# PhilippBongartz/RepeatResolver

Measured on AMD Instinct MI355X. Metric: sum-of-pairs DP cells/sec, higher is better.
Workload: dtype u32

## Files before the change

repeatresolver_amd/csrc/pwr_device.hip:

```cpp
#include <hip/hip_runtime.h>

#include <algorithm>
#include <chrono>
#include <cstdint>
#include <cstdio>
#include <cstdlib>
#include <cstring>
#include <new>
#include <thread>
#include <type_traits>
#include <vector>

#include "pwr.h"

#define PWR_INF 0x40000000u
#define PWR_BIG 0x7fffffff

struct Hdr {
    int W;
    int nslots;
    int nfree;
    int cur;
    int status;
    int stop;
// ... 990 lines not shown
                }
            } else {
                unsigned Mn[C];
                unsigned fa = 0;
#pragma unroll
                for (int i = 0; i < C; ++i) {
                    fa |= (tg[i] >= p) ? (1u << i) : 0u;
                    p = min(p, tg[i]);
                    Mn[i] = (rel0 + i < 0) ? PWR_INF : (unsigned)(gg[i] + p);
                }
                const unsigned mrow = needP ? ePy : PWR_INF;
                const unsigned left0 = (unsigned)__builtin_amdgcn_update_dpp((int)mrow, (int)Mn[C - 1], DPP_WAVE_SHR1, 0xF, 0xF, false);
#pragma unroll
                for (int i = 0; i < C; ++i) {
                    const unsigned lf = i ? Mn[i > 0 ? i - 1 : 0] : left0;
                    const bool inb = (unsigned)(rel0 + i) < (unsigned)Bx;
                    accA[i] = (accA[i] << 1) | ((((fa >> i) & 1u) || (inb && Mn[i] == lf)) ? 1u : 0u);
                    lastM[wave * MS + lc + i] = inb ? Mn[i] : 0xffffffffu;
                    Mprev[i] = Mn[i];
                }
            }
            nacc = (x & 15) + 1;
            if (lane == 63) {
                ST64(MBP(wave, x), P_end, x + 1);
                ST64(MBM(wave, x), Mprev[C - 1], x + 1);
                if (ms == ms_hi) ST64(PTB(x), P_end, x + 1);
            }
            ran_prev = 1;
            V2_NEXT_ROW()
        }
        if (lane == 0) __hip_atomic_store(&rdone[wave], round + 1, __ATOMIC_RELAXED, __HIP_MEMORY_SCOPE_WORKGROUP);
        __syncthreads();
        if (UNI(__hip_atomic_load(&s_done, __ATOMIC_RELAXED, __HIP_MEMORY_SCOPE_WORKGROUP)) >= NW) break;
    }
    if (round >= max_rounds) {
        if (tid == 0) { m->ok = 0; atomicCAS(&st.hdr->status, 0, PWR_ERR_INTERNAL); }
        return;
    }
    if (tid == 0) {
        m->clk = (unsigned)(__builtin_amdgcn_s_memtime() - t_clk0);
        m->rclk = (unsigned)(__builtin_amdgcn_s_memrealtime() - t_real0);
        m->rounds = round;
        atomicAdd(&st.hdr->cells_computed, m->cells);
    }
#undef MBP
#undef MBM
#undef PTB
#undef LD64
#undef LD32LO
#undef ST64
}

#ifndef PWR_INTERIOR_CLS
#define PWR_INTERIOR_CLS 0
#endif
#define V3_TICKS() ((unsigned)(__builtin_amdgcn_s_memtime() >> 10))
#define V3_TIMEOUT_TICKS (1u << 19)
#define V4_RB 128

#ifdef PWR_DIAG
#define DG_DECL unsigned long long dg_wait_fast = 0, dg_wait_gen = 0, dg_wait_setup = 0, dg_t = 0, dg_t2 = 0, dg_cyc_int = 0, dg_cyc_gen16 = 0, dg_ts1 = 0, dg_ts2 = 0, dg_tl2 = 0; unsigned dg_log = 0; unsigned dg_int = 0, dg_gen16 = 0, dg_general = 0, dg_nowork = 0, dg_runs = 0, dg_switch = 0;
#define DG_T0() dg_t = __builtin_amdgcn_s_memtime();
#define DG_ADD(ACC) ACC += __builtin_amdgcn_s_memtime() - dg_t;
#define DG_INC(CNT, N) CNT += (N);
#define DG_T2() dg_t2 = __builtin_amdgcn_s_memtime();
#define DG_ADD2(ACC) ACC += __builtin_amdgcn_s_memtime() - dg_t2;
#else
#define DG_T2()
#define DG_ADD2(ACC)
#define DG_DECL
#define DG_T0()
#define DG_ADD(ACC)
#define DG_INC(CNT, N)
#endif
template <int NW, int C, bool WG1>
__global__ __launch_bounds__(WG1 ? NW * 64 : 128) void k_fill_v3(DState st, JobBufs jb)
{
    constexpr int MS = 64 * C, RS = NW * MS;
    constexpr int NL = WG1 ? NW : 1;
    constexpr int RB = WG1 ? 64 : V4_RB;
    __shared__ __attribute__((aligned(16))) int ldsS1[NL][2][4][MS];
    __shared__ unsigned long long rP[NL][RB], rM[NL][RB];
    __shared__ int wprog[NL], wdone;
    const int vjob = WG1 ? (int)blockIdx.x : (int)(blockIdx.x + 8 * blockIdx.z), lane = threadIdx.x & 63;
    const int role = WG1 ? 0 : UNI((int)threadIdx.x >> 6);
    const int wave = WG1 ? UNI((int)threadIdx.x >> 6) : (int)blockIdx.y;
    const int lw = WG1 ? wave : 0, wr = WG1 ? (wave + 1) % NW : 0;
    if (vjob >= jb.njobs_launched * jb.smax) return;
    const int job = vjob / jb.smax;
    const SegDesc *const sd = jb.seg + (size_t)job * SEG_MAX + (vjob % jb.smax);
    JobMeta *m = &jb.meta[job];
    if (st.hdr->fallback > 0 && jb.v2_follows) return;
    if (!m->active || m->L <= 0 || !m->ok || m->wide || !sd->active || NOT_MINE(jb, job)) return;
    const int seg_xb = UNI(sd->xb), seg_fin = UNI(sd->fin);
    const int L = UNI(sd->xe) - seg_xb;
    const int Lf = seg_fin ? L - 1 : L;
    const int x_own = UNI(sd->xown) - seg_xb;
    const int g_own = x_own >> 4;
    const int chkA = x_own > 0 ? x_own : -1, chkB = seg_fin ? -1 : L;
    unsigned *const chk_w = jb.chk + (((size_t)job * (SEG_MAX + 1) + sd->s) * 2 + 0) * (size_t)jb.NC;
    unsigned *const chk_t = jb.chk + (((size_t)job * (SEG_MAX + 1) + sd->s + 1) * 2 + 1) * (size_t)jb.NC;
    const unsigned long long t_clk0 = __builtin_amdgcn_s_memtime(), t_real0 = __builtin_amdgcn_s_memrealtime();
    for (int i = threadIdx.x; i < NL * RB; i += blockDim.x) { (&rP[0][0])[i] = 0; (&rM[0][0])[i] = 0; }
    if (threadIdx.x < NL) wprog[threadIdx.x] = 0;
    if (threadIdx.x == 0) wdone = 0;
    __syncthreads();

    const int wl = (wave + NW - 1) % NW;
    const unsigned tagbase = jb.tagbase;
    const size_t gstride = (size_t)jb.gstride;
    unsigned long long *const gmy = jb.gmb + (((size_t)job * NW + wave) * gstride + (size_t)sd->grow0) * 2;
    const unsigned long long *const gleftw = jb.gmb + (((size_t)job * NW + wl) * gstride + (size_t)sd->grow0) * 2;
    const unsigned long long *const gjob = jb.gmb + ((size_t)job * NW * gstride + (size_t)sd->grow0) * 2;
#define PTOT_PTR(AP, BP, R) (gjob + (((size_t)((((AP) + (BP) - 1 - lo) / MS) % NW)) * gstride + (size_t)(R)) * 2)
    int *const abortf = &m->abort;
#define GLD(PTR) __hip_atomic_load((PTR), __ATOMIC_RELAXED, __HIP_MEMORY_SCOPE_AGENT)
#define GST(PTR, VAL, ROW) __hip_atomic_store((PTR), ((unsigned long long)(tagbase | (unsigned)((ROW) + 1)) << 32) | (unsigned)(VAL), __ATOMIC_RELAXED, __HIP_MEMORY_SCOPE_AGENT)
#define GST2(PTR, VAL, TAG) __hip_atomic_store((PTR), ((unsigned long long)(TAG) << 32) | (unsigned)(VAL), __ATOMIC_RELAXED, __HIP_MEMORY_SCOPE_AGENT)
#define TAGOF(W64) ((unsigned)((W64) >> 32))
#define LLD(REF) __hip_atomic_load(&(REF), __ATOMIC_RELAXED, __HIP_MEMORY_SCOPE_WORKGROUP)
#define LST(REF, V) __hip_atomic_store(&(REF), (V), __ATOMIC_RELAXED, __HIP_MEMORY_SCOPE_WORKGROUP)

    if (!WG1 && role == 1) {
        for (unsigned it = 0;; ++it) {
            if (UNI(LLD(wdone))) break;
            const int wx = UNI(LLD(wprog[lw]));
            const int r = wx - 1 + lane;
            const bool inr = r >= 0 && r < L;
            unsigned long long p = 0, q = 0;
            int ab = 0;
            if (inr) { p = GLD(gleftw + 2 * (size_t)r); q = GLD(gleftw + 2 * (size_t)r + 1); }
            if ((it & 15u) == 15u) ab = GLD(abortf);
            if (inr) {
                const unsigned tagr = tagbase | (unsigned)(r + 1);
                if (TAGOF(p) == tagr && TAGOF(q) == tagr) {
                    LST(rP[lw][r & (RB - 1)], p);
                    __hip_atomic_store(&rM[lw][r & (RB - 1)], q, __ATOMIC_RELEASE, __HIP_MEMORY_SCOPE_WORKGROUP);
                }
            }
            if (UNI(ab)) break;
        }
        return;
    }

    const int lo = UNI(m->lo), hi = UNI(m->hi), W = UNI(m->W), B = st.B, H = st.H;
    const int *way = jb.way + (size_t)job * jb.Lmax + seg_xb;
    const uint8_t *seq = st.seq + st.rowoff[UNI(m->k)] + seg_xb;
    const int4 *rec2 = jb.rec2 + (size_t)job * jb.colcap * 2;
    uint32_t *dirs = jb.dirs + (size_t)job * jb.dirstride + (size_t)(seg_xb >> 4) * RS;
    unsigned *lastM = jb.lastM + (size_t)job * jb.NC;
    const int lc = lane * C;
#define V4_LOADS(MSX, SLOT, AU, AG, AI, GL)                                                      \
    {                                                                                            \
        _Pragma("unroll") for (int i = 0; i < C; ++i) {                                          \
            const int y_ = lo + (MSX) * MS + lc + i;                                             \
            int4 p_ = make_int4(PWR_BIG / 2, PWR_BIG / 2, PWR_BIG / 2, PWR_BIG / 2);             \
            int4 q_ = make_int4(PWR_BIG / 2, 0, PWR_BIG / 2, 0);                                 \
            if (y_ <= hi) { p_ = rec2[2 * (y_ - lo)]; q_ = rec2[2 * (y_ - lo) + 1]; }            \
            ldsS1[lw][SLOT][0][lc + i] = p_.x; ldsS1[lw][SLOT][1][lc + i] = p_.y;                        \
            ldsS1[lw][SLOT][2][lc + i] = p_.z; ldsS1[lw][SLOT][3][lc + i] = p_.w;                        \
            AU[i] = q_.x; AG[i] = q_.y; AI[i] = q_.z;                                            \
        }                                                                                        \
        const int yq_ = lo + (MSX) * MS - 1;                                                     \
        GL = (yq_ >= lo && yq_ <= hi) ? UNI(rec2[2 * (yq_ - lo) + 1].y) : 0;                     \
    }

    int ug[C], gg[C], ig[C];
    int nu[C], ng[C], ni[C];
    int gleft = 0, gleftn = 0;
    const int ms_first = (max(0, UNI(way[0]) - H) - lo) / MS;
    int ms = ms_first + (((wave - ms_first) % NW) + NW) % NW, msn = ms + NW;
    int cs = 0;
    V4_LOADS(ms, 0, ug, gg, ig, gleft)
    V4_LOADS(msn, 1, nu, ng, ni, gleftn)

    const int src_prev = (seg_xb > 0 && jb.src_start) ? UNI(way[-1]) : -1;
    const int src_c = src_prev >= max(0, UNI(way[0]) - H) ? src_prev : -1;
    unsigned Mprev[C], accA[C], accC[C];
#pragma unroll
    for (int i = 0; i < C; ++i) { Mprev[i] = (src_c < 0 || lo + ms * MS + lc + i == src_c) ? 0u : PWR_INF; accA[i] = accC[i] = 0; }
    int gacc = -1, nacc = 0;
    int ran_prev = 0;
    int x = 0, blk = 0;
    int wcur = way[min(lane, L - 1)], scur = seq[min(lane, L - 1)];
    int wnxt = way[min(64 + lane, L - 1)], snxt = seq[min(64 + lane, L - 1)];
    const uint4 *desc = jb.desc + (size_t)job * jb.Lmax + seg_xb;
    const int fsh = 4 * (wave & 7);
    const unsigned *descw = (const unsigned *)desc + 1 + (wave >> 3);
    unsigned dca = desc[min(lane, L - 1)].x, dcf = descw[4 * min(lane, L - 1)] >> fsh;
    unsigned dna = desc[min(64 + lane, L - 1)].x, dnf = descw[4 * min(64 + lane, L - 1)];
    int a = max(0, __builtin_amdgcn_readlane(wcur, 0) - H), a_prev = 0, Bx_prev = 0;
    int sx = __builtin_amdgcn_readlane(scur, 0);

#define V4_CHK_STORE(XNEXT, AF, BEND)                                                            \
    if ((XNEXT) == chkA || (XNEXT) == chkB) {                                                    \
        unsigned *cv_ = (XNEXT) == chkA ? chk_w : chk_t;                                         \
        _Pragma("unroll") for (int i = 0; i < C; ++i) {                                          \
            const int y_ = lo + ms * MS + lc + i;                                                \
            cv_[wave * MS + lc + i] = (y_ >= (AF) && y_ < (BEND)) ? Mprev[i] : 0xffffffffu;      \
        }                                                                                        \
    }
#define V4_ALIGN_ACC(WANT)                                                                       \
    if (nacc != (WANT)) {                                                                        \
        const int sh_ = (WANT) - nacc;                                                           \
        _Pragma("unroll") for (int i = 0; i < C; ++i) { accA[i] <<= sh_; accC[i] <<= sh_; }      \
        nacc = (WANT);                                                                           \
    }
#define V4_FLUSH()                                                                               \
    if (gacc >= 0) {                                                                             \
        V4_ALIGN_ACC(16)                                                                         \
        uint32_t *d_ = dirs + (size_t)gacc * RS + (size_t)wave * MS + (size_t)lc;                \
        _Pragma("unroll") for (int i = 0; i < C; ++i) { if (gacc >= g_own) d_[i] = accA[i] | (accC[i] << 16); accA[i] = accC[i] = 0; } \
        gacc = -1; nacc = 0;                                                                     \
    }
#define V4_ROTATE_BLOCK()                                                                        \
    {                                                                                            \
        blk = x >> 6;                                                                            \
        wcur = wnxt; scur = snxt; dca = dna; dcf = dnf >> fsh;     \
        wnxt = way[min(x + 64 + lane, L - 1)];                                                   \
        snxt = seq[min(x + 64 + lane, L - 1)];                                                   \
        dna = desc[min(x + 64 + lane, L - 1)].x; dnf = descw[4 * min(x + 64 + lane, L - 1)];     \
    }
#define V4_NEXT_ROW()                                                                            \
    {                                                                                            \
        a_prev = a; Bx_prev = Bx;                                                                \
        ++x;                                                                                     \
        if (lane == 0) LST(wprog[lw], x);                                                            \
        if (x < L) {                                                                             \
            if ((x >> 6) != blk) V4_ROTATE_BLOCK()                                               \
            a = max(0, __builtin_amdgcn_readlane(wcur, x & 63) - H);                             \
            sx = __builtin_amdgcn_readlane(scur, x & 63);                                        \
        }                                                                                        \
    }

    DG_DECL
#ifdef PWR_DIAG
    unsigned long long *const tl = jb.diag + ((size_t)job * 32 + 31) * 4096 + (size_t)(sd->s * NW + wave) * 6;
    if (lane == 0 && sd->s * NW + wave < 680) { tl[0] = t_real0; tl[1] = __builtin_amdgcn_s_memrealtime(); tl[2] = 0; }
#endif
#define V4_EARLY_MASKS()                                                                         \
    if (early_hi >= (blk << 6)) {                                                                \
        const int b0_ = blk << 6;                                                                \
        const int lo_ = max(early_lo, b0_) - b0_, hi_ = min(early_hi, b0_ + 64) - b0_;           \
        const unsigned long long me_ = hi_ > lo_ ? ((hi_ - lo_ >= 64 ? ~0ull : ((1ull << (hi_ - lo_)) - 1ull)) << lo_) : 0ull; \
        const unsigned long long mf_ = early_hi < b0_ + 64 ? 1ull << (early_hi - b0_) : 0ull;    \
        bOm |= me_ | mf_; bMm |= me_ | mf_; bPm |= me_; bTm |= me_;                              \
    }
    bool dead = jb.stall_test && vjob == 0 && wave == 0;
    int first_pending = 0;
    int early_lo = 0, early_hi = -1;
    while (x < L && !dead) {
        ran_prev = UNI(ran_prev); gacc = UNI(gacc); nacc = UNI(nacc); blk = UNI(blk); ms = UNI(ms); cs = UNI(cs); gleft = UNI(gleft);
        x = UNI(x);
#ifdef PWR_DIAG
        if (ran_prev && !dg_tl2) { dg_tl2 = __builtin_amdgcn_s_memrealtime(); if (lane == 0 && sd->s * NW + wave < 680) { tl[2] = dg_tl2; tl[5] = (unsigned long long)x; } }
#endif
        if ((ran_prev || first_pending) && x < Lf) {
            unsigned long long bOm = __builtin_amdgcn_ballot_w64((dcf & 1u) != 0);
            const bool first = UNI(first_pending) != 0;
            if (first || ((bOm >> (x & 63)) & 1ull)) {
                first_pending = 0;
                unsigned long long bPm = __builtin_amdgcn_ballot_w64((dcf & 2u) != 0);
                unsigned long long bMm = __builtin_amdgcn_ballot_w64((dcf & 4u) != 0);
                unsigned long long bTm = __builtin_amdgcn_ballot_w64((dcf & 8u) != 0);
                if (first) { bOm |= 1ull << (x & 63); bMm |= 1ull << (x & 63); }
                V4_EARLY_MASKS()
                int dcaf = (int)(dca & 0xffffffu), dcb = min(dcaf + B, W);
                unsigned dcs = min(dca >> 24, 3u) * (unsigned)(MS * 4);
                if ((x >> 4) != gacc) { V4_FLUSH() gacc = x >> 4; }
                V4_ALIGN_ACC(x & 15)
                if (lane == 0) LST(wprog[lw], x);
                unsigned mlast_v = 0;
                if (first) {
                    const unsigned tagp = tagbase | (unsigned)x;
                    const int yq = lo + ms * MS - 1;
                    const bool needM = yq >= a_prev && yq < a_prev + Bx_prev;
                    unsigned long long eT = 0, eM = 0;
                    DG_T0()
#ifdef PWR_DIAG
                    const unsigned long long ev_t0 = __builtin_amdgcn_s_memrealtime();
#endif
                    const unsigned t0 = V3_TICKS();
                    for (unsigned spin = 1;; ++spin) {
                        eT = GLD(PTOT_PTR(a_prev, Bx_prev, x - 1));
                        eM = LLD(rM[lw][(x - 1) & (RB - 1)]);
                        if (UNI(TAGOF(eT)) == tagp && (!needM || UNI(TAGOF(eM)) == tagp)) break;
                        if ((spin & 1023u) == 0 && (V3_TICKS() - t0 > V3_TIMEOUT_TICKS || UNI(GLD(abortf)))) { dead = true; break; }
                        __builtin_amdgcn_s_sleep(1);
                    }
                    DG_ADD(dg_wait_gen)
#ifdef PWR_DIAG
                    if (lane == 0 && dg_general < 36) {
                        unsigned long long *ev = jb.diag + ((size_t)job * 32 + wave) * 4096 + 16 + 3 * dg_general;
                        ev[0] = (unsigned long long)x; ev[1] = ev_t0; ev[2] = __builtin_amdgcn_s_memrealtime();
                    }
#endif
                    DG_INC(dg_general, 1)
                    if (dead) break;
                    const int eTx = (int)UNI((unsigned)eT);
#pragma unroll
                    for (int i = 0; i < C; ++i) Mprev[i] = (unsigned)(gg[i] + eTx);
                    mlast_v = yq < a_prev ? PWR_INF : (needM ? UNI((unsigned)eM) : (unsigned)(gleft + eTx));
                    ran_prev = 1;
                } else if ((bMm >> (x & 63)) & 1ull) {
                    const unsigned tagp = tagbase | (unsigned)x;
                    unsigned long long w_ = LLD(rM[lw][(x - 1) & (RB - 1)]);
                    if (UNI(TAGOF(w_)) != tagp) {
                        DG_T0()
                        const unsigned t0 = V3_TICKS();
                        for (unsigned spin = 1;; ++spin) {
                            w_ = LLD(rM[lw][(x - 1) & (RB - 1)]);
                            if (UNI(TAGOF(w_)) == tagp) break;
                            if ((spin & 1023u) == 0 && (V3_TICKS() - t0 > V3_TIMEOUT_TICKS || UNI(GLD(abortf)))) { dead = true; break; }
                            __builtin_amdgcn_s_sleep(1);
                        }
                        DG_ADD(dg_wait_setup)
                        if (dead) break;
                    }
                    mlast_v = (unsigned)w_;
                }
                int ycol[C];
#pragma unroll
                for (int i = 0; i < C; ++i) ycol[i] = lo + ms * MS + lc + i;
                const char *const stab = (const char *)&ldsS1[lw][cs][0][lc];
                int sgr[C];
                {
                    const int *const srow0 = (const int *)(stab + __builtin_amdgcn_readlane((int)dcs, x & 63));
#pragma unroll
                    for (int i = 0; i < C; ++i) sgr[i] = srow0[i];
                }
                int af_done = a_prev;
                int g_af = 0, g_be = 0, g_cs = 0, g_cp = -1;
                DG_INC(dg_runs, 1)
                while (true) {
                    const int r_beg = x & 15, g0 = x - r_beg, r0 = g0 & 63;
                    int nrun = __builtin_ctz(~((unsigned)(bOm >> (r0 + r_beg)) & 0xffffu) | (1u << (16 - r_beg)));
                    nrun = min(nrun, Lf - x);
                    if (nrun <= 0) break;
                    const unsigned nPm = (unsigned)(bPm >> r0) & 0xffffu, kMm = (unsigned)(bMm >> r0) & 0xffffu, eTm = (unsigned)(bTm >> r0) & 0xffffu;
                    const unsigned p0 = (nPm >> r_beg) & 1u, m0 = (kMm >> r_beg) & 1u, t0_ = (eTm >> r_beg) & 1u;
                    const unsigned diff = ((nPm ^ (0u - p0)) | (kMm ^ (0u - m0)) | ((p0 & m0) ? 0u : (eTm ^ (0u - t0_)))) & 0xffffu;
                    const int nsame = __builtin_ctz((diff >> r_beg) | 0x10000u);
                    const bool mixed16 = r_beg == 0 && nrun == 16 && nsame < 16;
                    const int r_e = mixed16 ? 16 : r_beg + min(nrun, nsame);
                    const unsigned et_here = (eTm >> r_beg) & ((1u << (r_e - r_beg)) - 1u);
                    const int cls = mixed16 ? 3 : ((p0 & m0) ? (et_here ? 1 : 0) : ((p0 | m0 | t0_) == 0u ? 2 : 3));
                    if (gacc < 0) gacc = x >> 4;
#ifdef PWR_DIAG
                    if (!dg_ts1 && x >= 1024) dg_ts1 = __builtin_amdgcn_s_memrealtime();
                    if (!dg_ts2 && x >= 2048) dg_ts2 = __builtin_amdgcn_s_memrealtime();
#endif
                    if (WG1) {
                        const int need = g0 + 16 - RB + 2;
                        if (need > 0 && UNI(LLD(wprog[wr])) < need) {
                            DG_T0()
                            const unsigned t0 = V3_TICKS();
                            for (unsigned spin = 1;; ++spin) {
                                if (UNI(LLD(wprog[wr])) >= need) break;
                                if ((spin & 1023u) == 0 && (V3_TICKS() - t0 > V3_TIMEOUT_TICKS || UNI(GLD(abortf)))) { dead = true; break; }
                                __builtin_amdgcn_s_sleep(1);
                            }
                            DG_ADD(dg_wait_setup)
                            if (dead) break;
                        }
                    }
                    unsigned long long *const gq0 = gmy + 2 * (size_t)g0;
                    const unsigned tag_g0 = tagbase | (unsigned)g0;
                    const unsigned long long *const ringM = &rM[lw][g0 & (RB - 1)], *const ringP = &rP[lw][g0 & (RB - 1)];
                    if (g0 != g_cp) {
                        const int src = 4 * min(r0 + lane, 63);
                        g_af = __builtin_amdgcn_ds_bpermute(src, dcaf);
                        g_be = __builtin_amdgcn_ds_bpermute(src, dcb);
                        g_cs = __builtin_amdgcn_ds_bpermute(src, (int)dcs);
                        g_cp = g0;
                    }
                    auto group_row = [&](const int r, auto cls_, auto bits_) __attribute__((always_inline)) {
                        constexpr int CLS = decltype(cls_)::value;
                        constexpr bool BITS = decltype(bits_)::value;
                        bool bP = CLS <= 1 || CLS == 4, bM = CLS <= 1 || CLS == 4;
                        if (CLS == 3) { bP = (nPm >> r) & 1u; bM = (kMm >> r) & 1u; }
                        int af = 0, bend = 0;
                        if (CLS >= 2) af = __builtin_amdgcn_readlane(g_af, r);
                        if (CLS == 1 || CLS == 3 || CLS == 4) bend = __builtin_amdgcn_readlane(g_be, r);
                        const int Mleft_v = bM ? (int)mlast_v : (int)PWR_INF;
                        const int pm1_0 = __builtin_amdgcn_update_dpp(Mleft_v, (int)Mprev[C - 1], DPP_WAVE_SHR1, 0xF, 0xF, false);
                        int tg[C];
                        int run = FBIG;
#pragma unroll
                        for (int i = 0; i < C; ++i) {
                            const int pm1 = i ? (int)Mprev[i > 0 ? i - 1 : 0] : pm1_0;
                            const int d = pm1 + sgr[i];
                            const int u = (int)Mprev[i] + ug[i];
                            if (BITS) accC[i] = acc_push(accC[i], __builtin_amdgcn_sicmp(d, u, ICMP_SLE));
                            const int t3 = min(min(d, u), ig[i]);
                            bool inb = true;
                            if (CLS == 1 || CLS == 4) inb = ycol[i] < bend;
                            if (CLS == 2) inb = ycol[i] >= af;
                            if (CLS == 3) inb = (unsigned)(ycol[i] - af) < (unsigned)(bend - af);
                            tg[i] = inb ? t3 : FBIG;
                            run = min(run, tg[i]);
                        }
                        unsigned long long fM = 0;
                        unsigned fP = 0;
                        if (CLS != 2) {
                            fM = LLD(ringM[r]);
                            __builtin_amdgcn_sched_barrier(0);
                            fP = __hip_atomic_load((const unsigned *)&ringP[r], __ATOMIC_RELAXED, __HIP_MEMORY_SCOPE_WORKGROUP);
                        }
                        __builtin_amdgcn_sched_barrier(0);
#define V4_SCAN_STEP(CTRL, RMASK) { const int t_ = __builtin_amdgcn_update_dpp(PWR_BIG, incl, CTRL, RMASK, 0xF, false); incl = min(incl, t_); }
#define V4_FENCE() __builtin_amdgcn_sched_barrier(0)
                        int incl = run;
                        V4_SCAN_STEP(DPP_ROW_SHR(1), 0xF) V4_FENCE();
                        const int soff = __builtin_amdgcn_readlane(g_cs, r + 1);
                        V4_FENCE(); V4_SCAN_STEP(DPP_ROW_SHR(2), 0xF) V4_FENCE();
                        const int *const srow = (const int *)(stab + soff);
                        V4_FENCE(); V4_SCAN_STEP(DPP_ROW_SHR(4), 0xF) V4_FENCE();
#pragma unroll
                        for (int i = 0; i < C; ++i) sgr[i] = srow[i];
                        V4_FENCE(); V4_SCAN_STEP(DPP_ROW_SHR(8), 0xF) V4_FENCE();
                        const unsigned tagx = tag_g0 + (unsigned)(r + 1);
                        V4_FENCE(); V4_SCAN_STEP(DPP_ROW_BCAST15, 0xA) V4_FENCE();
                        V4_FENCE(); V4_SCAN_STEP(DPP_ROW_BCAST31, 0xC) V4_FENCE();
#undef V4_SCAN_STEP
#undef V4_FENCE
                        if (bP && __builtin_expect(UNI(TAGOF(fM)) != tagx, 0)) {
                            DG_T0()
                            const unsigned t0 = V3_TICKS();
                            for (unsigned spin = 1; !dead; ++spin) {
                                fM = LLD(ringM[r]);
                                __builtin_amdgcn_sched_barrier(0);
                                fP = __hip_atomic_load((const unsigned *)&ringP[r], __ATOMIC_RELAXED, __HIP_MEMORY_SCOPE_WORKGROUP);
                                if (UNI(TAGOF(fM)) == tagx) break;
                                if ((spin & 1023u) == 0 && (V3_TICKS() - t0 > V3_TIMEOUT_TICKS || UNI(GLD(abortf)))) { dead = true; break; }
                                __builtin_amdgcn_s_sleep(1);
                            }
                            DG_ADD(dg_wait_fast)
                        }
                        const int P_in_v = bP ? (int)fP : PWR_BIG;
                        const int P_end_v = min(P_in_v, incl);
                        const int pq = min(P_in_v, FBIG);
                        int p = min(__builtin_amdgcn_update_dpp(pq, incl, DPP_WAVE_SHR1, 0xF, 0xF, false), pq);
#pragma unroll
                        for (int i = 0; i < C; ++i) {
                            if (BITS) accA[i] = acc_push(accA[i], __builtin_amdgcn_sicmp(tg[i], p, ICMP_SGE));
                            p = min(p, tg[i]);
                            Mprev[i] = min((unsigned)(gg[i] + p), PWR_INF);
                        }
                        mlast_v = (unsigned)fM;
                        if (lane == 63) {
                            if (WG1) {
                                GST2(gq0 + 2 * r, P_end_v, tagx);
                                LST(rP[wr][(g0 + r) & (RB - 1)], ((unsigned long long)tagx << 32) | (unsigned)P_end_v);
                                LST(rM[wr][(g0 + r) & (RB - 1)], ((unsigned long long)tagx << 32) | (unsigned)Mprev[C - 1]);
                            } else {
                                typedef unsigned v4u_ __attribute__((ext_vector_type(4)));
                                v4u_ w4_; w4_.x = (unsigned)P_end_v; w4_.y = tagx; w4_.z = Mprev[C - 1]; w4_.w = tagx;
                                asm volatile("global_store_dwordx4 %0, %1, off sc1\n\ts_nop 1" :: "v"(gq0 + 2 * r), "v"(w4_) : "memory");
                            }
                        }
                    };
                    int r_end = r_e;
                    DG_T2()
                    using WithBits = std::integral_constant<bool, true>;
                    using NoBits = std::integral_constant<bool, false>;
                    const bool warmup = (x >> 4) < g_own;
                    if (warmup && r_beg == 0 && r_e == 16 && cls != 3) {
                        if (cls == 0) {
#pragma unroll
                            for (int r = 0; r < 16; ++r) group_row(r, std::integral_constant<int, PWR_INTERIOR_CLS>{}, NoBits{});
                            DG_INC(dg_int, 16)
                            DG_ADD2(dg_cyc_int)
                        } else if (cls == 1) {
#pragma unroll
                            for (int r = 0; r < 16; ++r) group_row(r, std::integral_constant<int, 1>{}, NoBits{});
                        } else {
#pragma unroll
                            for (int r = 0; r < 16; ++r) group_row(r, std::integral_constant<int, 2>{}, NoBits{});
                        }
                    } else if (cls == 0 && r_beg == 0 && r_e == 16) {
#pragma unroll
                        for (int r = 0; r < 16; ++r) group_row(r, std::integral_constant<int, PWR_INTERIOR_CLS>{}, WithBits{});
                        DG_INC(dg_int, 16)
                        DG_ADD2(dg_cyc_int)
                    } else if (cls == 1 && r_beg == 0 && r_e == 16) {
#pragma unroll
                        for (int r = 0; r < 16; ++r) group_row(r, std::integral_constant<int, 1>{}, WithBits{});
                    } else if (cls == 3 && r_beg == 0 && r_e == 16) {
#pragma unroll
                        for (int r = 0; r < 16; ++r) group_row(r, std::integral_constant<int, 3>{}, WithBits{});
                    } else if (cls == 2 && r_beg == 0 && r_e == 16) {
#pragma unroll
                        for (int r = 0; r < 16; ++r) group_row(r, std::integral_constant<int, 2>{}, WithBits{});
                    } else {
                        int r = r_beg;
                        for (; r < r_end && (r & 3) && !dead; ++r) group_row(r, std::integral_constant<int, 3>{}, WithBits{});
#define V4_BLOCKS(K) for (; r + 4 <= r_end && !dead; r += 4) { group_row(r, std::integral_constant<int, K>{}, WithBits{}); group_row(r + 1, std::integral_constant<int, K>{}, WithBits{}); \
                                                               group_row(r + 2, std::integral_constant<int, K>{}, WithBits{}); group_row(r + 3, std::integral_constant<int, K>{}, WithBits{}); }
                        if (cls == 0) V4_BLOCKS(0)
                        else if (cls == 1) V4_BLOCKS(1)
                        else if (cls == 2) V4_BLOCKS(2)
#undef V4_BLOCKS
                        for (; r < r_end && !dead; ++r) group_row(r, std::integral_constant<int, 3>{}, WithBits{});
                        r_end = r;
                    }
                    if (!(cls == 0 && r_beg == 0 && r_e == 16)) { DG_INC(dg_gen16, r_end - r_beg) DG_ADD2(dg_cyc_gen16) }
                    x = g0 + r_end;
#ifdef PWR_DIAG
                    if (lane == 0 && dg_log < 1270) {
                        unsigned long long *lg = jb.diag + ((size_t)job * 32 + wave) * 4096 + 256 + 3 * dg_log;
                        lg[0] = (unsigned long long)x | ((unsigned long long)cls << 32) | ((unsigned long long)(r_end - r_beg) << 40); lg[1] = __builtin_amdgcn_s_memrealtime();
                        lg[2] = dg_wait_fast + dg_wait_gen + dg_wait_setup;
                    }
                    dg_log += 1;
#endif
                    af_done = __builtin_amdgcn_readlane(dcaf, (x - 1) & 63);
                    if ((x & 15) == 0) {
                        uint32_t *d_ = dirs + (size_t)gacc * RS + (size_t)wave * MS + (size_t)lc;
#pragma unroll
                        for (int i = 0; i < C; ++i) { if (gacc >= g_own) d_[i] = accA[i] | (accC[i] << 16); accA[i] = accC[i] = 0; }
                        gacc = -1; nacc = 0;
                        V4_CHK_STORE(x, af_done, min(af_done + B, W))
                    } else nacc = x & 15;
                    if (dead || x >= Lf) break;
                    if ((x >> 6) != blk) {
                        V4_ROTATE_BLOCK()
                        bOm = __builtin_amdgcn_ballot_w64((dcf & 1u) != 0); bPm = __builtin_amdgcn_ballot_w64((dcf & 2u) != 0);
                        bMm = __builtin_amdgcn_ballot_w64((dcf & 4u) != 0); bTm = __builtin_amdgcn_ballot_w64((dcf & 8u) != 0);
                        V4_EARLY_MASKS()
                        dcaf = (int)(dca & 0xffffffu); dcb = min(dcaf + B, W);
                        dcs = min(dca >> 24, 3u) * (unsigned)(MS * 4);
                        g_cp = -1;
                        const int *const srow0 = (const int *)(stab + __builtin_amdgcn_readlane((int)dcs, 0));
#pragma unroll
                        for (int i = 0; i < C; ++i) sgr[i] = srow0[i];
                    }
                    if (lane == 0) LST(wprog[lw], x);
                }
                a_prev = af_done; Bx_prev = min(B, W - af_done);
                if (dead) break;
                if (x < L) {
                    if ((x >> 6) != blk) V4_ROTATE_BLOCK()
                    a = max(0, __builtin_amdgcn_readlane(wcur, x & 63) - H);
                    sx = __builtin_amdgcn_readlane(scur, x & 63);
                }
                if (lane == 0) LST(wprog[lw], x);
                continue;
            }
        }
        if (dead || x >= L) break;

        x = UNI(x); ms = UNI(ms); msn = UNI(msn); a = UNI(a); a_prev = UNI(a_prev); Bx_prev = UNI(Bx_prev);
        sx = UNI(sx); gacc = UNI(gacc); nacc = UNI(nacc); blk = UNI(blk); gleft = UNI(gleft); gleftn = UNI(gleftn); ran_prev = UNI(ran_prev); cs = UNI(cs);
        const int Bx = min(B, W - a);
        const int ms_lo = (a - lo) / MS, ms_hi = (a + Bx - 1 - lo) / MS;
        if (ms < ms_lo) {
            ms += NW;
            if (ms == msn) {
#pragma unroll
                for (int i = 0; i < C; ++i) { ug[i] = nu[i]; gg[i] = ng[i]; ig[i] = ni[i]; }
                gleft = gleftn;
                cs ^= 1;
            } else {
                while (ms < ms_lo) ms += NW;
                V4_LOADS(ms, cs, ug, gg, ig, gleft)
            }
            DG_INC(dg_switch, 1)
            msn = ms + NW;
            V4_LOADS(msn, cs ^ 1, nu, ng, ni, gleftn)
            ran_prev = 0;
            continue;
        }
        if (ms > ms_hi) {
            const int y0s = lo + ms * MS;
            const int anf_l = (int)(dca & 0xffffffu);
            const unsigned long long wm = __builtin_amdgcn_ballot_w64(min(anf_l + B, W) > y0s) >> (x & 63);
            const int xn = min(wm ? x + __builtin_ctzll(wm) : ((x >> 6) + 1) << 6, L);
            int xs = xn;
            if (wm && xn < Lf) {
                const int anf_up = __builtin_amdgcn_update_dpp(0x3fffffff, anf_l, DPP_WAVE_SHR1, 0xF, 0xF, false);
                const unsigned long long tears = __builtin_amdgcn_ballot_w64(anf_l >= min(anf_up + B, W)) >> (x & 63);
                const unsigned long long tm = tears & (~0ull >> (63 - (xn - x))) & ~1ull;
                xs = max(x, xn & ~15);
                if (tm) xs = max(xs, x + 63 - __builtin_clzll(tm));
                if (xs < 1) xs = xn;
                const int an = __builtin_amdgcn_readlane(anf_l, xn & 63);
                if (ms < (an - lo) / MS) { xs = xn; first_pending = 0; }
                else { early_lo = xs; early_hi = xn; first_pending = xs > 0 ? 1 : 0; }
            }
            DG_INC(dg_nowork, xs - x)
            if (xs > x) {
                const int al = __builtin_amdgcn_readlane((int)dca, (xs - 1) & 63) & 0xffffff;
                a_prev = al; Bx_prev = min(B, W - al);
            }
            x = xs;
            ran_prev = 0;
            if (lane == 0) LST(wprog[lw], x);
            if (x < L) {
                if ((x >> 6) != blk) V4_ROTATE_BLOCK()
                a = max(0, __builtin_amdgcn_readlane(wcur, x & 63) - H);
                sx = __builtin_amdgcn_readlane(scur, x & 63);
            }
            continue;
        }
        if (!ran_prev && x > 0 && x < Lf) { first_pending = 1; continue; }
        const int y0 = lo + ms * MS;
        const int yq = y0 - 1;
        const bool needP = ms > ms_lo;
        const bool needM = x > 0 && yq >= a_prev && yq < a_prev + Bx_prev;
        const bool needT = x > 0 && ((yq >= a_prev + Bx_prev) || !ran_prev);
        unsigned ePx = 0, ePy = 0, eMy = 0, eTx = 0;
        if (WG1 && x - RB + 2 > 0) {
            const unsigned t0 = V3_TICKS();
            for (unsigned spin = 1; UNI(LLD(wprog[wr])) < x - RB + 2; ++spin) {
                if ((spin & 1023u) == 0 && (V3_TICKS() - t0 > V3_TIMEOUT_TICKS || UNI(GLD(abortf)))) { dead = true; break; }
                __builtin_amdgcn_s_sleep(1);
            }
            if (dead) break;
        }
        {
            const unsigned tagx = tagbase | (unsigned)(x + 1), tagp = tagbase | (unsigned)x;
#ifdef PWR_DIAG
            const unsigned long long ev_t0 = __builtin_amdgcn_s_memrealtime();
#endif
            DG_T0()
            const unsigned t0 = V3_TICKS();
            for (unsigned spin = 1;; ++spin) {
                const unsigned long long eQ = LLD(rM[lw][x & (RB - 1)]), eP = LLD(rP[lw][x & (RB - 1)]);
                const unsigned long long eM = LLD(rM[lw][(x - 1) & (RB - 1)]), eT = needT ? GLD(PTOT_PTR(a_prev, Bx_prev, x - 1)) : 0ull;
                ePx = UNI((unsigned)eP); ePy = UNI((unsigned)eQ); eMy = UNI((unsigned)eM); eTx = UNI((unsigned)eT);
                const bool ready = (!needP || (UNI(TAGOF(eP)) == tagx && UNI(TAGOF(eQ)) == tagx)) &&
                                   (!needM || UNI(TAGOF(eM)) == tagp) && (!needT || UNI(TAGOF(eT)) == tagp);
                if (ready) break;
                if ((spin & 1023u) == 0 && (V3_TICKS() - t0 > V3_TIMEOUT_TICKS || UNI(GLD(abortf)))) { dead = true; break; }
                __builtin_amdgcn_s_sleep(1);
            }
#ifdef PWR_DIAG
            if (lane == 0 && dg_general < 36) {
                unsigned long long *ev = jb.diag + ((size_t)job * 32 + wave) * 4096 + 16 + 3 * dg_general;
                ev[0] = (unsigned long long)x; ev[1] = ev_t0; ev[2] = __builtin_amdgcn_s_memrealtime();
            }
#endif
            DG_ADD(dg_wait_gen)
            DG_INC(dg_general, 1)
            if (dead) break;
        }
        int Mleft = (int)PWR_INF;
        if (x == 0) Mleft = (src_c < 0 || yq == src_c) ? 0 : (int)PWR_INF;
        else if (yq < a_prev) Mleft = (int)PWR_INF;
        else if (needM) Mleft = (int)eMy;
        else Mleft = gleft + (int)eTx;
        const int P_in = needP ? (int)ePx : PWR_BIG;
        if (x > 0 && !ran_prev) {
#pragma unroll
            for (int i = 0; i < C; ++i) Mprev[i] = (unsigned)(gg[i] + (int)eTx);
        }
        if ((x >> 4) != gacc) { V4_FLUSH() gacc = x >> 4; }
        V4_ALIGN_ACC(x & 15)
        const int pm1_0 = __builtin_amdgcn_update_dpp(Mleft, (int)Mprev[C - 1], DPP_WAVE_SHR1, 0xF, 0xF, false);
        const int sxc = min(max(sx, 0), 3);
        const int rel0 = y0 + lc - a;
        int tg[C];
        int run = PWR_BIG;
#pragma unroll
        for (int i = 0; i < C; ++i) {
            const int pm1 = i ? (int)Mprev[i > 0 ? i - 1 : 0] : pm1_0;
            const int d = pm1 + ldsS1[lw][cs][sxc][lc + i];
            const int u = (int)Mprev[i] + ug[i];
            accC[i] = (accC[i] << 1) | ((d <= u) ? 1u : 0u);
            const int t3 = min(min(d, u), ig[i]);
            tg[i] = ((unsigned)(rel0 + i) < (unsigned)Bx) ? t3 : PWR_BIG;
            run = min(run, tg[i]);
        }
        const int incl = wave_incl_min(run);
        const int excl = __builtin_amdgcn_update_dpp(PWR_BIG, incl, DPP_WAVE_SHR1, 0xF, 0xF, false);
        const int P_end = min(P_in, __builtin_amdgcn_readlane(incl, 63));
        int p = min(P_in, excl);
        if (x != Lf) {
#pragma unroll
            for (int i = 0; i < C; ++i) {
                accA[i] = (accA[i] << 1) | ((tg[i] >= p) ? 1u : 0u);
                p = min(p, tg[i]);
                Mprev[i] = (rel0 + i < 0) ? PWR_INF : (unsigned)(gg[i] + p);
            }
        } else {
            unsigned Mn[C];
            unsigned fa = 0;
#pragma unroll
            for (int i = 0; i < C; ++i) {
                fa |= (tg[i] >= p) ? (1u << i) : 0u;
                p = min(p, tg[i]);
                Mn[i] = (rel0 + i < 0) ? PWR_INF : (unsigned)(gg[i] + p);
            }
            const unsigned mrow = needP ? ePy : PWR_INF;
            const unsigned left0 = (unsigned)__builtin_amdgcn_update_dpp((int)mrow, (int)Mn[C - 1], DPP_WAVE_SHR1, 0xF, 0xF, false);
#pragma unroll
            for (int i = 0; i < C; ++i) {
                const unsigned lf = i ? Mn[i > 0 ? i - 1 : 0] : left0;
                const bool inb = (unsigned)(rel0 + i) < (unsigned)Bx;
                accA[i] = (accA[i] << 1) | ((((fa >> i) & 1u) || (inb && Mn[i] == lf)) ? 1u : 0u);
                lastM[wave * MS + lc + i] = inb ? Mn[i] : 0xffffffffu;
                Mprev[i] = Mn[i];
            }
        }
        nacc = (x & 15) + 1;
        if (lane == 63) {
            GST(gmy + 2 * (size_t)x, P_end, x);
            if (WG1) {
                const unsigned long long tg_ = (unsigned long long)(tagbase | (unsigned)(x + 1)) << 32;
                LST(rP[wr][x & (RB - 1)], tg_ | (unsigned)P_end);
                LST(rM[wr][x & (RB - 1)], tg_ | (unsigned)Mprev[C - 1]);
            } else GST(gmy + 2 * (size_t)x + 1, Mprev[C - 1], x);
        }
        ran_prev = 1;
        V4_CHK_STORE(x + 1, a, a + Bx)
        V4_NEXT_ROW()
    }
    V4_FLUSH()
#ifdef PWR_DIAG
    if (lane == 0) {
        unsigned long long *dgp = jb.diag + ((size_t)job * 32 + wave) * 4096;
        dgp[0] = __builtin_amdgcn_s_memtime() - t_clk0; dgp[1] = dg_wait_fast; dgp[2] = dg_wait_gen; dgp[3] = dg_wait_setup;
        dgp[4] = ((unsigned long long)dg_int << 32) | dg_gen16; dgp[5] = ((unsigned long long)dg_general << 32) | dg_nowork;
        dgp[6] = ((unsigned long long)dg_runs << 32) | dg_switch; dgp[7] = (unsigned long long)L;
        dgp[12] = dg_log; dgp[8] = dg_cyc_gen16; dgp[9] = dg_ts1; dgp[10] = dg_ts2; dgp[11] = dg_cyc_int;
    }
#endif
#ifdef PWR_DIAG
    if (lane == 0 && sd->s * NW + wave < 680) { tl[3] = __builtin_amdgcn_s_memrealtime(); tl[4] = (unsigned long long)L | ((unsigned long long)(dg_wait_fast + dg_wait_gen + dg_wait_setup) << 20); }
#endif
    if (lane == 0) { LST(wprog[lw], 0x7fffffff); LST(wdone, 1); }
    if (dead) {
        if (lane == 0) __hip_atomic_store(abortf, 1, __ATOMIC_RELAXED, __HIP_MEMORY_SCOPE_AGENT);
        return;
    }
    if (wave == 0 && lane == 0) {
        if (sd->s == 0) {
            m->clk = (unsigned)(__builtin_amdgcn_s_memtime() - t_clk0);
            m->rclk = (unsigned)(__builtin_amdgcn_s_memrealtime() - t_real0);
            m->rounds = 0;
        }
        atomicAdd(&st.hdr->cells_computed, sd->cells);
    }
#undef V4_CHK_STORE
#undef V4_EARLY_MASKS
#undef PTOT_PTR
#undef GLD
#undef GST
#undef GST2
#undef TAGOF
#undef LLD
#undef LST
#undef V4_LOADS
#undef V4_ALIGN_ACC
#undef V4_FLUSH
#undef V4_ROTATE_BLOCK
#undef V4_NEXT_ROW
}

__device__ __forceinline__ bool seg_check_applies(const DState &st, const JobBufs &jb, int job, const JobMeta *m)
{
    return m->active && m->L > 0 && m->ok && !m->wide && !m->abort && !(st.hdr->fallback > 0 && jb.v2_follows) && !NOT_MINE(jb, job) && m->nseg > 1;
}

__device__ __forceinline__ void seg_check_body(const DState &st, const JobBufs &jb, const int job, const int s, const int tid)
{
    __shared__ int s_min[4], s_max[4], s_bad;
    JobMeta *m = &jb.meta[job];
    if (!seg_check_applies(st, jb, job, m)) return;
    if (s >= m->nseg) return;
    const SegDesc *sd = jb.seg + (size_t)job * SEG_MAX + s;
    const int xr = sd->xown - 1;
    const int lo = m->lo, W = m->W, B = st.B, H = st.H, RS = jb.NC;
    const int a = max(0, jb.way[(size_t)job * jb.Lmax + xr] - H), Bx = min(B, W - a);
    unsigned *cw = jb.chk + (((size_t)job * (SEG_MAX + 1) + s) * 2 + 0) * (size_t)jb.NC;
    unsigned *ct = jb.chk + (((size_t)job * (SEG_MAX + 1) + s) * 2 + 1) * (size_t)jb.NC;
    if (tid == 0) s_bad = 0;
    __syncthreads();
    int dmin = INT_MAX, dmax = INT_MIN, bad = 0;
    for (int j = tid; j < Bx; j += 256) {
        const int idx = (a + j - lo) % RS;
        const unsigned vw = cw[idx], vt = ct[idx];
        if (vw == 0xffffffffu || vt == 0xffffffffu) bad = 1;
        else if ((vw >= PWR_INF) != (vt >= PWR_INF)) bad = 1;
        else if (vw < PWR_INF) { const int d = (int)(vw - vt); dmin = min(dmin, d); dmax = max(dmax, d); }
    }
    for (int o = 32; o > 0; o >>= 1) { dmin = min(dmin, __shfl_xor(dmin, o)); dmax = max(dmax, __shfl_xor(dmax, o)); }
    if ((tid & 63) == 0) { s_min[tid >> 6] = dmin; s_max[tid >> 6] = dmax; }
    if (bad) s_bad = 1;
    __syncthreads();
    for (int j = tid; j < RS; j += 256) { cw[j] = 0xffffffffu; ct[j] = 0xffffffffu; }
    if (tid == 0) {
        const int lo_ = min(min(s_min[0], s_min[1]), min(s_min[2], s_min[3])), hi_ = max(max(s_max[0], s_max[1]), max(s_max[2], s_max[3]));
        if (s_bad || (lo_ != INT_MAX && lo_ != hi_)) __hip_atomic_store(&m->segfail, 1, __ATOMIC_RELAXED, __HIP_MEMORY_SCOPE_AGENT);
        if (s == 1) { atomicAdd(&st.hdr->seg_jobs, 1ull); atomicAdd(&st.hdr->segs, (unsigned long long)m->nseg); }
        __hip_atomic_fetch_add(&jb.chkdone[job], 1, __ATOMIC_RELEASE, __HIP_MEMORY_SCOPE_AGENT);
    }
}

__global__ __launch_bounds__(256) void k_seg_check(DState st, JobBufs jb)
{
    seg_check_body(st, jb, (int)blockIdx.x, (int)blockIdx.y + 1, (int)threadIdx.x);
}

#define F64_NT 1024
#define F64_INF (1ll << 62)
__global__ __launch_bounds__(F64_NT) void k_fill64(DState st, JobBufs jb)
{
    __shared__ long long prevM[2][2 * F64_NT + 2];
    __shared__ long long wtot[F64_NT / 64];
    __shared__ long long s_lastcell[2], s_min;
    const int job = blockIdx.x, tid = threadIdx.x, lane = tid & 63, wv = tid >> 6;
    JobMeta *m = &jb.meta[job];
    const int L = m->L;
    if (!m->active || L <= 0 || !m->ok || !m->wide || NOT_MINE(jb, job)) return;
    const int lo = m->lo, hi = m->hi, W = m->W, B = st.B, H = st.H, RS = jb.NC;
    const int n = hi - lo + 1;
    const int *way = jb.way + (size_t)job * jb.Lmax;
    const uint8_t *seq = st.seq + st.rowoff[m->k];
    const uint8_t *mark = jb.mark + (size_t)job * jb.colcap;
    const int *order = cur_order(st);
    uint32_t *dirs = jb.dirs + (size_t)job * jb.dirstride;
    unsigned *lastM = jb.lastM + (size_t)job * jb.NC;
    long long *G = jb.g64 + (size_t)job * jb.colcap;
    const int way0 = way[0], wayL = way[L - 1];
    auto tally_of = [&](int y, uint32_t *w) {
        const Tally t = st.tally[order[y]];
#pragma unroll
        for (int b = 0; b < 6; ++b) w[b] = t.w[b];
        if (y >= way0 && y <= wayL) {
            const int mk = mark[y - lo];
            const int own = mk == 7 ? 5 : (mk ? mk - 1 : 4);
#pragma unroll
            for (int b = 0; b < 6; ++b) w[b] -= (own != 5 && b != own) ? 1u : 0u;
        }
    };
    {
        long long carry = 0;
        for (int base = 0; base < n; base += F64_NT) {
            const int i = base + tid;
            long long v = 0;
            if (i < n) { uint32_t w[6]; tally_of(lo + i, w); v = (long long)w[4]; }
            long long incl = v;
            for (int o = 1; o < 64; o <<= 1) { const long long t = __shfl_up(incl, o); if (lane >= o) incl += t; }
            if (lane == 63) wtot[wv] = incl;
            __syncthreads();
            long long pre = 0, tot = 0;
            for (int w = 0; w < F64_NT / 64; ++w) { const long long s = wtot[w]; pre += (w < wv) ? s : 0; tot += s; }
            __syncthreads();
            if (i < n) G[i] = carry + pre + incl;
            carry += tot;
        }
        const size_t nwords = (size_t)((L + 15) / 16) * RS;
        for (size_t i = tid; i < nwords; i += F64_NT) dirs[i] = 0;
        for (int i = tid; i < RS; i += F64_NT) lastM[i] = 0xffffffffu;
// ... 2819 lines not shown
```

Before: 53.36 billion.

## Store M values biased by gap cost to drop per-cell adds in inner loop

Changes the representation of Mprev to exclude the per-row gap term gg[i], folding that term into the preloaded substitution scores in LDS and into the up-gap costs. This removes the gg[i]+p add from each cell update in the hot DP row loop, and the boundary/left values are rebiased by gleft to match. The final row and checkpoint stores convert back to true M values. A store instruction is also changed to use an SGPR base with a VGPR offset. This shifts some work into the load phase and risks off-by-bias errors at the INF boundaries.

```diff
diff --git a/repeatresolver_amd/csrc/pwr_device.hip b/repeatresolver_amd/csrc/pwr_device.hip
--- a/repeatresolver_amd/csrc/pwr_device.hip
+++ b/repeatresolver_amd/csrc/pwr_device.hip
@@ -1166,17 +1166,23 @@
     const int lc = lane * C;
 #define V4_LOADS(MSX, SLOT, AU, AG, AI, GL)                                                      \
     {                                                                                            \
+        const int yq_ = lo + (MSX) * MS - 1;                                                     \
+        GL = (yq_ >= lo && yq_ <= hi) ? UNI(rec2[2 * (yq_ - lo) + 1].y) : 0;                     \
+        int4 p_[C];                                                                              \
         _Pragma("unroll") for (int i = 0; i < C; ++i) {                                          \
             const int y_ = lo + (MSX) * MS + lc + i;                                             \
-            int4 p_ = make_int4(PWR_BIG / 2, PWR_BIG / 2, PWR_BIG / 2, PWR_BIG / 2);             \
+            p_[i] = make_int4(PWR_BIG / 2, PWR_BIG / 2, PWR_BIG / 2, PWR_BIG / 2);               \
             int4 q_ = make_int4(PWR_BIG / 2, 0, PWR_BIG / 2, 0);                                 \
-            if (y_ <= hi) { p_ = rec2[2 * (y_ - lo)]; q_ = rec2[2 * (y_ - lo) + 1]; }            \
-            ldsS1[lw][SLOT][0][lc + i] = p_.x; ldsS1[lw][SLOT][1][lc + i] = p_.y;                        \
-            ldsS1[lw][SLOT][2][lc + i] = p_.z; ldsS1[lw][SLOT][3][lc + i] = p_.w;                        \
-            AU[i] = q_.x; AG[i] = q_.y; AI[i] = q_.z;                                            \
+            if (y_ <= hi) { p_[i] = rec2[2 * (y_ - lo)]; q_ = rec2[2 * (y_ - lo) + 1]; }         \
+            AU[i] = q_.x + q_.y; AG[i] = q_.y; AI[i] = q_.z;                                     \
         }                                                                                        \
-        const int yq_ = lo + (MSX) * MS - 1;                                                     \
-        GL = (yq_ >= lo && yq_ <= hi) ? UNI(rec2[2 * (yq_ - lo) + 1].y) : 0;                     \
+        const int gl0_ = __builtin_amdgcn_update_dpp(GL, AG[C - 1], DPP_WAVE_SHR1, 0xF, 0xF, false);   \
+        _Pragma("unroll") for (int i = 0; i < C; ++i) {                                          \
+            const int y_ = lo + (MSX) * MS + lc + i;                                             \
+            const int gp_ = y_ <= hi ? (i ? AG[i > 0 ? i - 1 : 0] : gl0_) : 0;                   \
+            ldsS1[lw][SLOT][0][lc + i] = p_[i].x + gp_; ldsS1[lw][SLOT][1][lc + i] = p_[i].y + gp_;      \
+            ldsS1[lw][SLOT][2][lc + i] = p_[i].z + gp_; ldsS1[lw][SLOT][3][lc + i] = p_[i].w + gp_;      \
+        }                                                                                        \
     }
 
     int ug[C], gg[C], ig[C];
@@ -1192,7 +1198,7 @@
     const int src_c = src_prev >= max(0, UNI(way[0]) - H) ? src_prev : -1;
     unsigned Mprev[C], accA[C], accC[C];
 #pragma unroll
-    for (int i = 0; i < C; ++i) { Mprev[i] = (src_c < 0 || lo + ms * MS + lc + i == src_c) ? 0u : PWR_INF; accA[i] = accC[i] = 0; }
+    for (int i = 0; i < C; ++i) { Mprev[i] = (unsigned)((src_c < 0 || lo + ms * MS + lc + i == src_c) ? -gg[i] : ig[i]); accA[i] = accC[i] = 0; }
     int gacc = -1, nacc = 0;
     int ran_prev = 0;
     int x = 0, blk = 0;
@@ -1211,7 +1217,7 @@
         unsigned *cv_ = (XNEXT) == chkA ? chk_w : chk_t;                                         \
         _Pragma("unroll") for (int i = 0; i < C; ++i) {                                          \
             const int y_ = lo + ms * MS + lc + i;                                                \
-            cv_[wave * MS + lc + i] = (y_ >= (AF) && y_ < (BEND)) ? Mprev[i] : 0xffffffffu;      \
+            cv_[wave * MS + lc + i] = (y_ >= (AF) && y_ < (BEND)) ? (unsigned)gg[i] + Mprev[i] : 0xffffffffu;    \
         }                                                                                        \
     }
 #define V4_ALIGN_ACC(WANT)                                                                       \
@@ -1313,8 +1319,8 @@
                     if (dead) break;
                     const int eTx = (int)UNI((unsigned)eT);
 #pragma unroll
-                    for (int i = 0; i < C; ++i) Mprev[i] = (unsigned)(gg[i] + eTx);
-                    mlast_v = yq < a_prev ? PWR_INF : (needM ? UNI((unsigned)eM) : (unsigned)(gleft + eTx));
+                    for (int i = 0; i < C; ++i) Mprev[i] = (unsigned)eTx;
+                    mlast_v = yq < a_prev ? PWR_INF - (unsigned)gleft : (needM ? UNI((unsigned)eM) : (unsigned)eTx);
                     ran_prev = 1;
                 } else if ((bMm >> (x & 63)) & 1ull) {
                     const unsigned tagp = tagbase | (unsigned)x;
@@ -1396,7 +1402,7 @@
                         int af = 0, bend = 0;
                         if (CLS >= 2) af = __builtin_amdgcn_readlane(g_af, r);
                         if (CLS == 1 || CLS == 3 || CLS == 4) bend = __builtin_amdgcn_readlane(g_be, r);
-                        const int Mleft_v = bM ? (int)mlast_v : (int)PWR_INF;
+                        const int Mleft_v = bM ? (int)mlast_v : (int)PWR_INF - gleft;
                         const int pm1_0 = __builtin_amdgcn_update_dpp(Mleft_v, (int)Mprev[C - 1], DPP_WAVE_SHR1, 0xF, 0xF, false);
                         int tg[C];
                         int run = FBIG;
@@ -1459,7 +1465,7 @@
                         for (int i = 0; i < C; ++i) {
                             if (BITS) accA[i] = acc_push(accA[i], __builtin_amdgcn_sicmp(tg[i], p, ICMP_SGE));
                             p = min(p, tg[i]);
-                            Mprev[i] = min((unsigned)(gg[i] + p), PWR_INF);
+                            Mprev[i] = (unsigned)(CLS == 0 ? p : min(p, ig[i]));
                         }
                         mlast_v = (unsigned)fM;
                         if (lane == 63) {
@@ -1470,7 +1476,7 @@
                             } else {
                                 typedef unsigned v4u_ __attribute__((ext_vector_type(4)));
                                 v4u_ w4_; w4_.x = (unsigned)P_end_v; w4_.y = tagx; w4_.z = Mprev[C - 1]; w4_.w = tagx;
-                                asm volatile("global_store_dwordx4 %0, %1, off sc1\n\ts_nop 1" :: "v"(gq0 + 2 * r), "v"(w4_) : "memory");
+                                asm volatile("global_store_dwordx4 %0, %1, %2 sc1\n\ts_nop 1" :: "v"(16 * r), "v"(w4_), "s"(gq0) : "memory");
                             }
                         }
                     };
@@ -1660,14 +1666,14 @@
             if (dead) break;
         }
         int Mleft = (int)PWR_INF;
-        if (x == 0) Mleft = (src_c < 0 || yq == src_c) ? 0 : (int)PWR_INF;
-        else if (yq < a_prev) Mleft = (int)PWR_INF;
+        if (x == 0) Mleft = (src_c < 0 || yq == src_c) ? -gleft : (int)PWR_INF - gleft;
+        else if (yq < a_prev) Mleft = (int)PWR_INF - gleft;
         else if (needM) Mleft = (int)eMy;
-        else Mleft = gleft + (int)eTx;
+        else Mleft = (int)eTx;
         const int P_in = needP ? (int)ePx : PWR_BIG;
         if (x > 0 && !ran_prev) {
 #pragma unroll
-            for (int i = 0; i < C; ++i) Mprev[i] = (unsigned)(gg[i] + (int)eTx);
+            for (int i = 0; i < C; ++i) Mprev[i] = eTx;
         }
         if ((x >> 4) != gacc) { V4_FLUSH() gacc = x >> 4; }
         V4_ALIGN_ACC(x & 15)
@@ -1695,7 +1701,7 @@
             for (int i = 0; i < C; ++i) {
                 accA[i] = (accA[i] << 1) | ((tg[i] >= p) ? 1u : 0u);
                 p = min(p, tg[i]);
-                Mprev[i] = (rel0 + i < 0) ? PWR_INF : (unsigned)(gg[i] + p);
+                Mprev[i] = (unsigned)((rel0 + i < 0) ? ig[i] : p);
             }
         } else {
             unsigned Mn[C];
@@ -1705,8 +1711,9 @@
                 fa |= (tg[i] >= p) ? (1u << i) : 0u;
                 p = min(p, tg[i]);
                 Mn[i] = (rel0 + i < 0) ? PWR_INF : (unsigned)(gg[i] + p);
-            }
-            const unsigned mrow = needP ? ePy : PWR_INF;
+                Mprev[i] = (unsigned)((rel0 + i < 0) ? ig[i] : p);
+            }
+            const unsigned mrow = needP ? (unsigned)gleft + ePy : PWR_INF;
             const unsigned left0 = (unsigned)__builtin_amdgcn_update_dpp((int)mrow, (int)Mn[C - 1], DPP_WAVE_SHR1, 0xF, 0xF, false);
 #pragma unroll
             for (int i = 0; i < C; ++i) {
@@ -1714,7 +1721,6 @@
                 const bool inb = (unsigned)(rel0 + i) < (unsigned)Bx;
                 accA[i] = (accA[i] << 1) | ((((fa >> i) & 1u) || (inb && Mn[i] == lf)) ? 1u : 0u);
                 lastM[wave * MS + lc + i] = inb ? Mn[i] : 0xffffffffu;
-                Mprev[i] = Mn[i];
             }
         }
         nacc = (x & 15) + 1;
```

New measurement: 55.06 billion, median of 6. 3.2% higher.
